# mohsenzakeri/Movi

Measured on AMD Instinct MI355X. Metric: PML query Gbases/s on regular-thresholds index, higher is better.
Workload: dtype u64

## Files before the change

movi_amd/csrc/movi_walk.hpp:

```cpp
#pragma once
#include "movi_device.hpp"

namespace movi {

template <int MODE, typename IdxT, int CLS, int SEP, int SEG, int STG, int AHD, int PSH, int RING>
__global__ __launch_bounds__(256) void pml_kernel_flatp(DevIndex ix, const uint8_t *__restrict__ bases,
                                                       const uint64_t *__restrict__ offs, uint64_t n_reads,
                                                       uint16_t *__restrict__ out, uint8_t *__restrict__ err,
                                                       DevStats *stats, const uint32_t *__restrict__ order,
                                                       ClsArgs cls, SegArgs seg) {
    static_assert(SEG == 0 || CLS == 0, "segments: plain PML");
    static_assert(AHD == 0 || STG == 1, "look-ahead rows: staged reads");
    static_assert(AHD == 0 || AHD == 1 || AHD == 2, "plain rows, look-ahead rows or deep rows");
    static_assert(AHD != 2 || (PSH == 0 && sizeof(IdxT) == 4), "deep rows: tables of fewer than 2^28 rows, no pair-shared gathers");
    static_assert(PSH == 0 || STG == 1, "pair-shared gathers: staged kernels");
    static_assert(RING == 0 || STG == 1, "PMLs out through the LDS ring / as reset masks: staged kernels");
    static_assert(RING != 2 || (CLS == 0 && SEG == 0), "reset masks: plain PML of whole reads");
    enum : uint32_t { sFF = 0, sDown = 1, sUp = 2, sDone = 3 };
    __shared__ uint8_t s_code[256];
    for (int i = threadIdx.x; i < 256; i += blockDim.x) s_code[i] = ix.code_of[i];
    __syncthreads();

    const uint64_t t = (uint64_t)blockIdx.x * blockDim.x + threadIdx.x;
    uint32_t ff_total = 0, scan_total = 0, repo_total = 0, failed = 0, err_total = 0;
    const EndThr ethr = end_thresholds(ix);
    const IdxT r1 = (IdxT)(ix.r - 1), end_row = (IdxT)ix.end_bwt_idx;
    const uint2 row_r1 = load_row<MODE>(ix.rows, r1);
    const uint32_t off0 = row_n<MODE>(row_r1) - 1;

    const bool valid = (SEG == 1 ? (*seg.go != 0u && t < *seg.n_seg) : (t < n_reads && (SEG != 2 || seg.read_fail[t] != 0)));
    const uint64_t rid = (valid && order && SEG == 0) ? order[t] : t;
    const uint64_t beg = valid ? (SEG == 1 ? seg.seg_in[rid] : offs[rid]) : 0;
    const uint32_t len = valid ? (SEG == 1 ? seg.seg_len[rid] : (uint32_t)(offs[rid + 1] - beg)) : 0;
    const uint64_t obeg = (SEG == 1 && valid) ? seg.seg_out[rid] : beg;
    constexpr bool ring = RING == 1;
    constexpr bool msk = RING == 2;
    uint32_t *const M = msk ? reinterpret_cast<uint32_t *>(out) + (((beg + ix.mask_phase) >> 5) + rid) : nullptr;
    uint32_t mk = 0;
    const uint32_t packed_end = len & (ring ? ~15u : ~7u);

    auto load_pair_at = [&](uint64_t e, uint64_t &c0, uint64_t &c1) {
        uint64_t two[2];
        __builtin_memcpy(two, bases + (e >= 16 ? e - 16 : 0), 16);
        c0 = two[1];
        c1 = two[0];
    };
    auto fix_pair = [&](uint64_t e, uint64_t &c0, uint64_t &c1) {
        if (e < 16) {
            const uint32_t sh = 8u * (uint32_t)(16 - e);
            if (sh >= 64) { c0 = c1 << (sh - 64); c1 = 0; }
            else { c0 = (c0 << sh) | (c1 >> (64 - sh)); c1 <<= sh; }
        }
    };
    constexpr uint32_t WN = 4u;
    const IdxT wb_last = (IdxT)(ix.r - WN);
    auto win_base = [&](IdxT nd) -> IdxT {
        const IdxT wb = nd & ~(IdxT)(WN - 1u);
        return wb < wb_last ? wb : wb_last;
    };
    uint2 ahw[4];
    uint4 raw[4];
    uint4 dq[4];
    const uint32_t odd_lane = threadIdx.x & 1u;
    auto fetch = [&](IdxT nd, bool act, uint2 (&w)[4]) {
        if (AHD == 2) {
            const uint32_t q3 = __umulhi((uint32_t)nd, 0xAAAAAAABu) >> 1;
            const uint8_t *at = ix.rows3 + (act ? (uint64_t)q3 * 64u : 0u);
            __builtin_memcpy(&dq[0], at, 16);
            __builtin_memcpy(&dq[1], at + 16, 16);
            __builtin_memcpy(&dq[2], at + 32, 16);
            __builtin_memcpy(&dq[3], at + 48, 16);
            return;
        }
        if (PSH) {
            uint64_t at;
            if (AHD) {
                const IdxT wb = nd & ~(IdxT)3;
                at = wb < wb_last ? (uint64_t)(wb >> 3) * 128u + (uint64_t)((uint32_t)wb & 4u) * 8u : ix.rows2_tail;
            } else {
                at = (uint64_t)win_base(nd) * 8u;
            }
            if (!act) at = 0;
            const uint64_t pat = (uint64_t)pair_swap((uint32_t)at) | ((uint64_t)pair_swap((uint32_t)(at >> 32)) << 32);
            const uint8_t *tab = AHD ? ix.rows2 : ix.rows;
            const uint8_t *pe = tab + (odd_lane ? pat : at) + 16u * odd_lane;
            const uint8_t *po = tab + (odd_lane ? at : pat) + 16u * odd_lane;
            __builtin_memcpy(&raw[0], pe, 16);
            if (AHD) __builtin_memcpy(&raw[2], pe + 64u, 16);
            __builtin_memcpy(&raw[1], po, 16);
            if (AHD) __builtin_memcpy(&raw[3], po + 64u, 16);
            return;
        }
        if (AHD) {
            const IdxT wb = nd & ~(IdxT)3;
            const bool body = wb < wb_last;
            uint64_t at = body ? (uint64_t)(wb >> 3) * 128u + (uint64_t)((uint32_t)wb & 4u) * 8u : ix.rows2_tail;
            if (!act) at = 0;
            load_window<MODE>(ix.rows2 + at, 0, w);
            load_window<MODE>(ix.rows2 + at + 64u, 0, ahw);
        } else {
            load_window<MODE>(ix.rows, (uint64_t)(act ? win_base(nd) : (IdxT)0), w);
        }
    };
    ClsState cs;
    auto finish_read = [&]() {
        if (SEG == 1) {
            SegTot tt;
            tt.ff = ff_total; tt.scan = scan_total; tt.repo = repo_total; tt.flag = failed;
            seg.tot[rid] = tt;
            return;
        }
        if (msk) {
            if (failed) {
                for (uint32_t wd = 0; wd * 32u < len; ++wd) M[wd] = (len - wd * 32u >= 32u) ? 0xFFFFFFFFu : ((1u << (len & 31u)) - 1u);
            } else if (len & 31u) {
                M[len >> 5] = mk;
            }
        } else if (failed && CLS != 2) {
            for (uint32_t i = 0; i < len; ++i) out[obeg + i] = 0;
        }
        if (CLS) cs.store(cls, rid, failed != 0u);
        if (err) err[rid] = (uint8_t)failed;
        err_total += failed ? 1u : 0u;
    };

    uint32_t st = len > 0 ? sFF : sDone;
    IdxT need = r1;
    uint32_t k = 0;
    uint32_t ml = 0, ff_run = 0;
    uint32_t off = off0;
    uint64_t rb = 0, rb2 = 0, nx0 = 0, nx1 = 0;
    if (st != sDone) {
        load_pair_at(beg + len, rb, rb2);
        fix_pair(beg + len, rb, rb2);
    }
    if (!STG && len > 16) load_pair_at(beg + len - 16, nx0, nx1);
    uint32_t a = s_code[(uint32_t)(rb >> 56) & 0xFFu];
    uint4 pk = make_uint4(0, 0, 0, 0), pk_old = pk;
    if (CLS) cs.init(len, cls.bin_width);
    extern __shared__ __align__(16) uint8_t s_stage[];
    uint8_t *const s_ring = s_stage + ix.stage_lds * 64u;
    const uint32_t ring_lane = (threadIdx.x & 63u) * 16u;
    auto ring_put = [&](uint32_t kk, uint32_t val) {
        *reinterpret_cast<uint16_t *>(s_ring + ((kk >> 3) & 3u) * 1024u + ring_lane + (kk & 7u) * 2u) = (uint16_t)val;
    };
    auto ring_flush = [&](uint32_t k0) {
        const uint32_t g = (k0 >> 4) & 1u;
        const uint4 lo = *reinterpret_cast<const uint4 *>(s_ring + (2u * g) * 1024u + ring_lane);
        const uint4 hi = *reinterpret_cast<const uint4 *>(s_ring + (2u * g + 1u) * 1024u + ring_lane);
        uint16_t *dst = out + obeg + (k0 & ~15u);
        __builtin_memcpy(dst, &lo, 16);
        __builtin_memcpy(dst + 8, &hi, 16);
    };
    uint32_t kbase = 0;
    const uint32_t stage_cap = ix.stage_lds;
#ifndef MOVI_STAGE_UNROLL
#define MOVI_STAGE_UNROLL 2
#endif
    constexpr uint32_t kStageUnroll = MOVI_STAGE_UNROLL;
    auto stage_from = [&](uint32_t k0, bool on) {
        uint32_t *S = reinterpret_cast<uint32_t *>(s_stage);
        const uint32_t sl = threadIdx.x & 63u;
        const uint32_t left = (on && len > k0) ? len - k0 : 0u;
        const uint32_t cnt = left < stage_cap ? left : stage_cap;
        for (uint32_t g = 0; wave_any(16u * g < cnt); g += kStageUnroll) {
            uint64_t c0[kStageUnroll], c1[kStageUnroll];
#pragma unroll
            for (uint32_t u = 0; u < kStageUnroll; ++u) {
                const uint64_t e = 16u * (g + u) < cnt ? beg + len - k0 - 16u * (g + u) : 16u;
                load_pair_at(e, c0[u], c1[u]);
            }
#pragma unroll
            for (uint32_t u = 0; u < kStageUnroll; ++u) {
                if (16u * (g + u) < cnt) {
                    const uint64_t e = beg + len - k0 - 16u * (g + u);
                    fix_pair(e, c0[u], c1[u]);
                    const uint64_t r0 = __builtin_bswap64(c0[u]), r1 = __builtin_bswap64(c1[u]);
                    S[(4u * (g + u) + 0u) * 64u + sl] = (uint32_t)r0;
                    S[(4u * (g + u) + 1u) * 64u + sl] = (uint32_t)(r0 >> 32);
                    S[(4u * (g + u) + 2u) * 64u + sl] = (uint32_t)r1;
                    S[(4u * (g + u) + 3u) * 64u + sl] = (uint32_t)(r1 >> 32);
                }
            }
        }
        if (on) kbase = k0;
    };
    auto staged_code = [&](uint32_t slot) -> uint32_t {
        const uint32_t q = slot < stage_cap ? slot : stage_cap - 1u;
        return s_code[s_stage[(q >> 2) * 256u + (threadIdx.x & 63u) * 4u + (q & 3u)]];
    };
    if (STG) stage_from(0u, st != sDone);
    auto top_of_walk = [&](uint32_t cand, uint32_t kidx) -> uint32_t {
        const uint32_t K = ix.kmer_k;
        uint4 e4 = make_uint4(0, 0, 0, 0);
        if (cand) e4 = ix.kmer[kidx];
        const uint32_t use = cand & (e4.y >> 31);
        if (msk) {
            if (use) {
                const uint32_t mask = (e4.y >> 16) & 0xFFFu;
                mk = ~mask & ((1u << K) - 1u);
                k = K;
                ml = (uint32_t)__builtin_clz(~(mask << (32u - K)));
                need = (IdxT)((uint64_t)e4.x | ((uint64_t)(e4.y & 15u) << 32));
                off = (e4.y >> 4) & 0xFFFu;
                ff_total += e4.z;
                scan_total += e4.w;
                repo_total += K - (uint32_t)__popc(mask);
            }
        } else if (use) {
            const uint32_t mask = (e4.y >> 16) & 0xFFFu;
            uint16_t *O = out + obeg;
            uint32_t run = 0;
            for (uint32_t i = 0; i < K; ++i) {
                run = ((mask >> i) & 1u) ? run + 1u : 0u;
                if (CLS) cs.add(run, k, len, cls.bin_width, cls.thr);
                if (CLS == 2) {
                } else if (k >= packed_end) {
                    O[k] = (uint16_t)run;
                } else if (STG && ring) {
                    ring_put(k, run);
                } else {
                    pk.x = (pk.x >> 16) | (pk.y << 16);
                    pk.y = (pk.y >> 16) | (pk.z << 16);
                    pk.z = (pk.z >> 16) | (pk.w << 16);
                    pk.w = (pk.w >> 16) | (run << 16);
                    if ((k & 15) == 7) {
                        if (k + 8 < packed_end) pk_old = pk;
                        else __builtin_memcpy(O + (k - 7), &pk, 16);
                    }
                }
                k += 1;
            }
            ml = run;
            need = (IdxT)((uint64_t)e4.x | ((uint64_t)(e4.y & 15u) << 32));
            off = (e4.y >> 4) & 0xFFFu;
            ff_total += e4.z;
            scan_total += e4.w;
            repo_total += K - (uint32_t)__popc(mask);
        }
        return use;
    };
    if (ix.kmer_k != 0u) {
        const uint32_t K = ix.kmer_k;
        uint32_t kidx = 0, bad = 0;
        for (uint32_t i = 0; i < K; ++i) {
            const uint64_t src = i < 8u ? rb : rb2;
            const uint32_t cc = (uint32_t)s_code[(uint32_t)(src >> (8u * (7u - (i & 7u)))) & 0xFFu] - (uint32_t)SEP;
            bad |= (uint32_t)(cc > 3u);
            kidx |= (cc & 3u) << (2u * i);
        }
        if (top_of_walk((uint32_t)(st != sDone) & (uint32_t)(len > K) & (bad ^ 1u), kidx)) {
            if (K >= 8u) rb = rb2;
            a = s_code[(uint32_t)(rb >> (8u * (7u - (K & 7u)))) & 0xFFu];
        }
    }
    uint32_t a1 = 0xFFu, a2 = 0xFFu;
    if (AHD) a1 = staged_code(k + 1);
    if (AHD == 2) a2 = staged_code(k + 2);
    uint2 w[4];
    fetch(need, st != sDone, w);

    uint32_t lane_steps = 0, wave_steps = 0;
    while (wave_any(st != sDone)) {
        const bool act = st < sDone;
        lane_steps += (uint32_t)act;
        wave_steps += 1;
#if defined(MOVI_PAD_PRE) && MOVI_PAD_PRE > 0
        {
            uint32_t pad = wave_steps;
#pragma unroll
            for (int i = 0; i < MOVI_PAD_PRE; ++i) asm volatile("v_add_u32 %0, %0, %0" : "+v"(pad));
        }
#endif
        struct StepOut {
            uint32_t resolved, match, ffm, lf, mism, scanning, found, down, qf, qn, jump, jdist, landed, landed_down, nf, n, rofff, emit;
            uint32_t dbl, lf2, off1, tpl, lf3, off2, errc, st_next;
            uint64_t j;
            IdxT needf, need_next, j2, j3;
        } R;
        R.tpl = 0; R.lf3 = 0; R.off2 = 0; R.j3 = 0;
        if (AHD == 2) {
            const uint32_t need32 = (uint32_t)need;
            const uint32_t wbase = (__umulhi(need32, 0xAAAAAAABu) >> 1) * 3u;
            const uint32_t r1u = (uint32_t)r1;
            const uint32_t d1a = dq[0].y, d1b = dq[1].z, d1c = dq[2].w;
            const uint32_t n0 = d1a & 0x7FFu, n1w = d1b & 0x7FFu, n2w = d1c & 0x7FFu;
            const uint32_t nm = (uint32_t)(((d1a >> 22) & 7u) != a) | ((uint32_t)(((d1b >> 22) & 7u) != a) << 1) | ((uint32_t)(((d1c >> 22) & 7u) != a) << 2);
            const uint32_t lim = r1u - wbase;
            const uint32_t first_win = (uint32_t)(wbase == 0u);
            uint32_t nd = need32;
            {
                const uint32_t q0 = nd - wbase;
                const uint32_t inw = (uint32_t)(q0 < 3u) & (uint32_t)(st < sDone);
                const uint32_t m0 = q0 == 0u, m1 = q0 <= 1u;
                const uint32_t t1 = m0 ? n0 : 0u, t2 = t1 + (m1 ? n1w : 0u), t3 = t2 + n2w;
                const uint32_t isff = inw & (uint32_t)(st == sFF);
                const uint32_t room = 65534u - (ff_run < 65534u ? ff_run : 65534u);
                uint32_t p0 = isff & m0 & (uint32_t)(off >= t1) & (uint32_t)(0u < lim), p1 = isff & m1 & (uint32_t)(off >= t2) & (uint32_t)(1u < lim),
                         p2 = isff & (uint32_t)(off >= t3) & (uint32_t)(2u < lim);
                uint32_t cf = p0 + p1 + p2;
                if (cf > room) {
                    cf = room;
                    const uint32_t first = m0 ? 0u : (m1 ? 1u : 2u);
                    p0 = p0 & (uint32_t)(first + cf > 0u);
                    p1 = p1 & (uint32_t)(first + cf > 1u);
                    p2 = p2 & (uint32_t)(first + cf > 2u);
                }
                off -= (p2 ? t3 : (p1 ? t2 : (p0 ? t1 : 0u)));
                ff_run += cf;
                const uint32_t dmask = (nm & (lim >= 3u ? 7u : ((1u << lim) - 1u))) >> q0;
                const uint32_t cd = (inw & (uint32_t)(st == sDown)) ? (uint32_t)__builtin_ctz(~dmask | 8u) : 0u;
                const uint32_t umask = ((nm & (first_win ? 6u : 7u)) << (2u - (q0 < 3u ? q0 : 2u))) & 7u;
                const uint32_t cu = (inw & (uint32_t)(st == sUp)) ? (uint32_t)__builtin_clz(((~umask) & 7u) << 29 | 0x10000000u) : 0u;
                scan_total += cd + cu;
                nd = nd + cf + cd - cu;
            }
            need = (IdxT)nd;
            const uint32_t qn = nd - wbase;
            const uint32_t inwin = (uint32_t)(qn < 3u) & (uint32_t)act;
            auto sel3 = [](uint32_t x0, uint32_t x1, uint32_t x2, uint32_t q) { return q == 0u ? x0 : (q == 1u ? x1 : x2); };
            const uint32_t rD0 = sel3(dq[0].x, dq[1].y, dq[2].z, qn), rD1 = sel3(d1a, d1b, d1c, qn);
            const uint32_t n = rD1 & 0x7FFu, c = (rD1 >> 22) & 7u;
            const uint32_t isFF = (uint32_t)(st == sFF) & inwin, isDown = (uint32_t)(st == sDown) & inwin, isUp = (uint32_t)(st == sUp) & inwin;
            const uint32_t ffm = isFF & (uint32_t)(nd < r1u) & (uint32_t)(off >= n);
            const uint32_t ff_over = ffm & (uint32_t)(ff_run + 1 >= 65535u);
            const uint32_t resolved = isFF & (ffm ^ 1u);
            const uint32_t illegal = a == 0xFFu, match = c == a;
            const uint32_t mism = resolved & (illegal ^ 1u) & (match ^ 1u);
            const uint32_t kk = thr_slot(SEP, a, c);
            const uint32_t kc = kk > 2u ? 2u : kk;
            uint32_t thr = ((rD0 >> (28u + kc)) & 1u) ? n : 0u;
            if (SEP) {
                if (mism & (uint32_t)(c == 0u) & (uint32_t)(need != end_row)) thr = separator_threshold(ix, (uint64_t)need, a);
            }
            const uint32_t down = (uint32_t)(off >= ((need == end_row) ? end_threshold(SEP, ethr, a) : thr));
            const uint32_t at_last = nd >= r1u, at_first = nd == 0u;
            const uint32_t repo_edge = mism & (down ? at_last : at_first);
            const uint32_t has = (nm ^ 7u) & (down ? (6u << qn) & 7u : (1u << qn) - 1u);
            const uint32_t found = mism & (uint32_t)(has != 0u) & ix.inwin;
            const uint32_t qf = found ? (down ? (uint32_t)__builtin_ctz(has | 8u) : 31u - (uint32_t)__builtin_clz(has | 1u)) : qn;
            const uint32_t far = mism & (found ^ 1u);
            const uint32_t f0 = sel3(dq[0].x, dq[1].y, dq[2].z, qf), f1 = sel3(d1a, d1b, d1c, qf), f2 = sel3(dq[0].z, dq[1].w, dq[3].x, qf),
                           f3 = sel3(dq[0].w, dq[2].x, dq[3].y, qf), f4 = sel3(dq[1].x, dq[2].y, dq[3].z, qf);
            const uint32_t fx = (dq[3].w >> (10u * (qf < 3u ? qf : 0u))) & 0x3FFu;
            const uint32_t nf = f1 & 0x7FFu, rofff = (f1 >> 11) & 0x7FFu;
            const uint32_t scanning = isDown | isUp;
            const uint32_t hit = scanning & match;
            const uint32_t landed = hit | found;
            const uint32_t landed_down = hit ? isDown : down;
            const uint32_t scan_edge = scanning & (hit ^ 1u) & (isDown ? at_last : at_first);
            const uint32_t emit = (resolved & (illegal | match)) | landed;
            const uint32_t lf = emit & (uint32_t)(k + 1 != len);
            const uint32_t jj = f0 & 0x0FFFFFFFu;
            const uint32_t lf_bad = lf & (uint32_t)(jj >= (uint32_t)ix.r);
            const uint32_t h6 = (f2 >> 28) | ((fx >> 8) << 4);
            const uint32_t hd = __builtin_amdgcn_ubfe(h6, kc + kc, ix.hint_w);
            const uint32_t jump = far & (uint32_t)(hd != 0u);
            const uint32_t jtgt = down ? wbase + 2u + hd : wbase - hd;
            const uint32_t jdist = down ? jtgt - nd : nd - jtgt;
            const uint32_t step_fwd = ffm | (far & down) | (scanning & (hit ^ 1u) & isDown);
            const uint32_t step_back = (far & (down ^ 1u)) | (scanning & (hit ^ 1u) & isUp);
            uint32_t need_next = lf ? jj : (jump ? jtgt : nd + step_fwd - step_back);
            uint32_t st_next = (emit & (lf ^ 1u)) ? sDone : (lf ? sFF : (far ? (down ? sDown : sUp) : st));
            const uint32_t e1n = f3 & 0x7FFu, e1off = (f3 >> 11) & 0x7FFu, e1c = (f1 >> 25) & 7u, jj2 = f2 & 0x0FFFFFFFu;
            const uint32_t e2n = (f3 >> 22) | (((f4 >> 28) & 1u) << 10), e2off = ((f4 >> 29) & 7u) | ((fx & 0xFFu) << 3), e2c = (f1 >> 28) & 7u,
                           jj3 = f4 & 0x0FFFFFFFu;
            const uint32_t off_e = (landed ? (landed_down ? 0u : nf - 1u) : off) + rofff;
            const uint32_t dbl = lf & (uint32_t)(a1 == e1c) & (uint32_t)(off_e < e1n);
            const uint32_t lf2 = dbl & (uint32_t)(k + 2 != len);
            const uint32_t off_e2 = off_e + e1off;
            const uint32_t tpl = lf2 & (uint32_t)(a2 == e2c) & (uint32_t)(off_e2 < e2n);
            const uint32_t lf3 = tpl & (uint32_t)(k + 3 != len);
            need_next = tpl ? (lf3 ? jj3 : nd) : (dbl ? (lf2 ? jj2 : nd) : need_next);
            st_next = tpl ? (lf3 ? sFF : sDone) : (dbl ? (lf2 ? sFF : sDone) : st_next);
            uint32_t errc = kErrNone;
            if (wave_any((ff_over | repo_edge | scan_edge | lf_bad) != 0u)) {
                errc = ff_over ? kErrFastForward
                               : (repo_edge ? (down ? kErrNoRunBelow : kErrNoRunAbove)
                                  : (scan_edge ? (isDown ? kErrNoRunBelow : kErrNoRunAbove)
                                     : (lf_bad ? kErrIdRange : kErrNone)));
                if (errc) { need_next = nd; st_next = sDone; }
            }
            R.resolved = resolved; R.match = match; R.ffm = ffm; R.lf = lf; R.mism = mism; R.scanning = scanning; R.found = found; R.down = down;
            R.qf = qf; R.qn = qn; R.jump = jump; R.jdist = jdist; R.landed = landed; R.landed_down = landed_down; R.nf = nf; R.n = n; R.rofff = rofff;
            R.emit = emit; R.dbl = dbl; R.lf2 = lf2; R.off1 = e1off; R.tpl = tpl; R.lf3 = lf3; R.off2 = e2off; R.errc = errc; R.st_next = st_next;
            R.j = jj; R.needf = (IdxT)(wbase + qf); R.need_next = (IdxT)need_next; R.j2 = (IdxT)jj2; R.j3 = (IdxT)jj3;
        } else {
            if (PSH) {
                pair_assemble(odd_lane, raw[0], raw[1], w);
                if (AHD) pair_assemble(odd_lane, raw[2], raw[3], ahw);
            }
            const IdxT wbase = win_base(need);
            auto hop = [&]() {
                const uint32_t q = (uint32_t)(need - wbase);
                const uint32_t inwin = (uint32_t)(q < WN) & (uint32_t)(st < sDone);
                const uint2 hr = win_sel(w, q);
                const uint32_t hn = row_n<MODE>(hr), hc = row_c<MODE>(hr);
                const uint32_t ffh = inwin & (uint32_t)(st == sFF) & (uint32_t)(need < r1) & (uint32_t)(off >= hn) &
                                     (uint32_t)(ff_run + 1 < 65535u);
                const uint32_t nomatch = hc != a;
                const uint32_t dnh = inwin & (uint32_t)(st == sDown) & nomatch & (uint32_t)(need < r1);
                const uint32_t uph = inwin & (uint32_t)(st == sUp) & nomatch & (uint32_t)(need != 0);
                off = ffh ? off - hn : off;
                ff_run += ffh;
                scan_total += dnh | uph;
                need = need + (IdxT)(ffh + dnh) - (IdxT)uph;
            };
            const uint32_t nm = (uint32_t)(row_c<MODE>(w[0]) != a) | ((uint32_t)(row_c<MODE>(w[1]) != a) << 1) |
                                ((uint32_t)(row_c<MODE>(w[2]) != a) << 2) | ((uint32_t)(row_c<MODE>(w[3]) != a) << 3);
            const uint32_t last_win = (uint32_t)(wbase + 3 == r1);
            const uint32_t first_win = (uint32_t)(wbase == 0);
            auto window_advance = [&]() {
                const uint32_t q0 = (uint32_t)(need - wbase);
                const uint32_t inwin = (uint32_t)(q0 < 4u) & (uint32_t)(st < sDone);
                const uint32_t n0 = row_n<MODE>(w[0]), n1 = row_n<MODE>(w[1]), n2 = row_n<MODE>(w[2]), n3 = row_n<MODE>(w[3]);
                const uint32_t m0 = q0 == 0u, m1 = q0 <= 1u, m2 = q0 <= 2u;
                const uint32_t t1 = m0 ? n0 : 0u, t2 = t1 + (m1 ? n1 : 0u), t3 = t2 + (m2 ? n2 : 0u), t4 = t3 + n3;
                const uint32_t isff = inwin & (uint32_t)(st == sFF);
                const uint32_t p0 = isff & m0 & (uint32_t)(off >= t1), p1 = isff & m1 & (uint32_t)(off >= t2),
                               p2 = isff & m2 & (uint32_t)(off >= t3), p3 = isff & (uint32_t)(off >= t4) & (last_win ^ 1u);
                const uint32_t cf = p0 + p1 + p2 + p3;
                off -= (p3 ? t4 : (p2 ? t3 : (p1 ? t2 : (p0 ? t1 : 0u))));
                ff_run += cf;
                const uint32_t dmask = (nm & (last_win ? 7u : 15u)) >> (q0 & 3u);
                const uint32_t cd = (inwin & (uint32_t)(st == sDown)) ? (uint32_t)__builtin_ctz(~dmask | 16u) : 0u;
                const uint32_t umask = ((nm & (first_win ? 14u : 15u)) << (3u - (q0 & 3u))) & 15u;
                const uint32_t cu = (inwin & (uint32_t)(st == sUp)) ? (uint32_t)__builtin_clz(((~umask) & 15u) << 28 | 0x08000000u) : 0u;
                scan_total += cd + cu;
                need = need + (IdxT)(cf + cd) - (IdxT)cu;
            };
            if (wave_any(st == sFF && ff_run >= 65520u)) {
                for (int h = 0; h < 4; ++h) hop();
            } else {
                window_advance();
            }
            const uint32_t qn = (uint32_t)(need - wbase);
            const uint32_t inwin = (uint32_t)(qn < WN) & (uint32_t)act;
            const uint2 row = win_sel(w, qn);
            const uint32_t n = row_n<MODE>(row), c = row_c<MODE>(row);
            const uint32_t isFF = (uint32_t)(st == sFF) & inwin, isDown = (uint32_t)(st == sDown) & inwin,
                           isUp = (uint32_t)(st == sUp) & inwin;
            const uint32_t ffm = isFF & (uint32_t)(need < r1) & (uint32_t)(off >= n);
            const uint32_t ff_over = ffm & (uint32_t)(ff_run + 1 >= 65535u);
            const uint32_t resolved = isFF & (ffm ^ 1u);
            const uint32_t illegal = a == 0xFFu, match = c == a;
            const uint32_t mism = resolved & (illegal ^ 1u) & (match ^ 1u);
            const uint32_t kk = thr_slot(SEP, a, c);
            uint32_t thr = row_thr<MODE>(row, kk > 2u ? 2u : kk) ? n : 0u;
            if (SEP) {
                if (mism & (uint32_t)(c == 0u) & (uint32_t)(need != end_row)) thr = separator_threshold(ix, (uint64_t)need, a);
            }
            const uint32_t down = (uint32_t)(off >= ((need == end_row) ? end_threshold(SEP, ethr, a) : thr));
            const uint32_t at_last = need >= r1, at_first = need == 0;
            const uint32_t repo_edge = mism & (down ? at_last : at_first);
            const uint32_t has = (nm ^ 15u) & (down ? (14u << (qn & 3u)) & 15u : (1u << (qn & 3u)) - 1u);
            const uint32_t found = mism & (uint32_t)(has != 0u) & ix.inwin;
            const uint32_t qf = found ? (down ? (uint32_t)__builtin_ctz(has | 16u) : 31u - (uint32_t)__builtin_clz(has | 1u)) : qn;
            const uint32_t far = mism & (found ^ 1u);
            const uint2 rowf = win_sel(w, qf);
            const uint32_t nf = row_n<MODE>(rowf), rofff = row_off<MODE>(rowf);
            const IdxT needf = (IdxT)(wbase + qf);
            const uint32_t scanning = isDown | isUp;
            const uint32_t hit = scanning & match;
            const uint32_t landed = hit | found;
            const uint32_t landed_down = hit ? isDown : down;
            const uint32_t scan_edge = scanning & (hit ^ 1u) & (isDown ? at_last : at_first);
            const uint32_t emit = (resolved & (illegal | match)) | landed;
            const uint32_t lf = emit & (uint32_t)(k + 1 != len);
            constexpr bool id32 = AHD != 0 && sizeof(IdxT) == 4;
            uint64_t j = 0;
            if (id32) j = (uint64_t)rowf.x;
            else if (MODE == 6 || lf) j = (AHD && ix.hints) ? (uint64_t)rowf.x : row_id<MODE>(rowf, needf, ix);
            const uint32_t lf_bad = lf & (uint32_t)(j >= ix.r);
            uint2 ah = make_uint2(0u, 0u);
            if (AHD) ah = win_sel(ahw, qf);
            uint32_t jump = 0, jdist = 0;
            IdxT jtgt = 0;
            if (AHD) {
                const uint32_t hbits = (rowf.y >> 28) | ((ah.y >> 21) & 0x3F0u);
                const uint32_t kc = kk > 2u ? 2u : kk;
                const uint32_t hd = __builtin_amdgcn_ubfe(hbits, kc + 2u * kc, ix.hint_w);
                jump = far & (uint32_t)(hd != 0u);
                jtgt = down ? (IdxT)(wbase + 3u + hd) : (IdxT)(wbase - hd);
                jdist = down ? (uint32_t)(jtgt - need) : (uint32_t)(need - jtgt);
            }
            const uint32_t step_fwd = ffm | (far & down) | (scanning & (hit ^ 1u) & isDown);
            const uint32_t step_back = (far & (down ^ 1u)) | (scanning & (hit ^ 1u) & isUp);
            IdxT need_next = lf ? (IdxT)j : (jump ? jtgt : (IdxT)(need + step_fwd - step_back));
            uint32_t st_next = (emit & (lf ^ 1u)) ? sDone : (lf ? sFF : (far ? (down ? sDown : sUp) : st));
            uint32_t dbl = 0, lf2 = 0, off1 = 0;
            IdxT j2 = 0;
            if (AHD) {
                const uint32_t n1 = ah.y & 0x7FFu, c1 = (ah.y >> 22) & 7u;
                const uint32_t off_e = (landed ? (landed_down ? 0u : nf - 1u) : off) + rofff;
                dbl = lf & (ah.y >> 31) & (uint32_t)(a1 == c1) & (uint32_t)(off_e < n1);
                lf2 = dbl & (uint32_t)(k + 2 != len);
                off1 = (ah.y >> 11) & 0x7FFu;
                j2 = (id32 || ix.hints) ? (IdxT)ah.x : (IdxT)((uint64_t)ah.x | ((uint64_t)((ah.y >> 25) & 15u) << 32));
                need_next = dbl ? (lf2 ? j2 : need) : need_next;
                st_next = dbl ? (lf2 ? sFF : sDone) : st_next;
            }
            uint32_t errc = kErrNone;
            if (wave_any((ff_over | repo_edge | scan_edge | lf_bad) != 0u)) {
                errc = ff_over ? kErrFastForward
                               : (repo_edge ? (down ? kErrNoRunBelow : kErrNoRunAbove)
                                  : (scan_edge ? (isDown ? kErrNoRunBelow : kErrNoRunAbove)
                                     : (lf_bad ? kErrIdRange : kErrNone)));
                if (errc) { need_next = need; st_next = sDone; }
            }
            R.resolved = resolved; R.match = match; R.ffm = ffm; R.lf = lf; R.mism = mism; R.scanning = scanning; R.found = found; R.down = down;
            R.qf = qf; R.qn = qn; R.jump = jump; R.jdist = jdist; R.landed = landed; R.landed_down = landed_down; R.nf = nf; R.n = n; R.rofff = rofff;
            R.emit = emit; R.dbl = dbl; R.lf2 = lf2; R.off1 = off1; R.errc = errc; R.st_next = st_next;
            R.j = j; R.needf = needf; R.need_next = need_next; R.j2 = j2;
        }
        const uint32_t resolved = R.resolved, match = R.match, ffm = R.ffm, lf = R.lf, mism = R.mism, scanning = R.scanning, found = R.found,
                       down = R.down, qf = R.qf, qn = R.qn, jump = R.jump, jdist = R.jdist, landed = R.landed, landed_down = R.landed_down,
                       nf = R.nf, n = R.n, rofff = R.rofff, emit = R.emit, dbl = R.dbl, lf2 = R.lf2, off1 = R.off1, tpl = R.tpl, lf3 = R.lf3,
                       off2 = R.off2, errc = R.errc, st_next = R.st_next;
        const uint64_t j = R.j;
        const IdxT needf = R.needf, need_next = R.need_next, j2 = R.j2, j3 = R.j3;
        (void)j3; (void)tpl; (void)lf3; (void)off2;
        fetch(need_next, st_next != sDone, w);
#if defined(MOVI_PAD_POST) && MOVI_PAD_POST > 0
        {
            uint32_t pad = wave_steps;
#pragma unroll
            for (int i = 0; i < MOVI_PAD_POST; ++i) asm volatile("v_add_u32 %0, %0, %0" : "+v"(pad));
        }
#endif
        uint32_t want_nx = 0;
        uint64_t nx_e = 0;
        ml = resolved ? (match ? ml + 1 : 0u) : ml;
        ff_total += resolved ? ff_run : 0u;
        ff_run = lf ? 0u : ff_run + ffm;
        repo_total += mism;
        scan_total += scanning + (found ? (down ? qf - qn : qn - qf) : 0u) + (jump ? jdist - 1u : 0u);
        off = ffm ? off - n : (landed ? (landed_down ? 0u : nf - 1) : off);
        const uint32_t off_pre = off;
        off += lf ? rofff : 0u;
        if (emit) {
            uint16_t *O = out + obeg;
            auto emit_pml = [&](uint32_t mlv) {
                const uint32_t val = mlv > 65535u ? 65535u : mlv;
                if (CLS) cs.add(val, k, len, cls.bin_width, cls.thr);
                if (CLS == 2) {
                } else if (msk) {
                    mk |= (uint32_t)(mlv == 0u) << (k & 31u);
                    if ((k & 31u) == 31u) { M[k >> 5] = mk; mk = 0u; }
                } else if (k >= packed_end) {
                    O[k] = (uint16_t)val;
                } else if (STG && ring) {
                    ring_put(k, val);
                } else {
                    pk.x = (pk.x >> 16) | (pk.y << 16);
                    pk.y = (pk.y >> 16) | (pk.z << 16);
                    pk.z = (pk.z >> 16) | (pk.w << 16);
                    pk.w = (pk.w >> 16) | (val << 16);
                    if ((k & 15) == 7) {
                        if (k + 8 < packed_end) pk_old = pk;
                        else __builtin_memcpy(O + (k - 7), &pk, 16);
                    } else if ((k & 15) == 15) {
                        __builtin_memcpy(O + (k - 15), &pk_old, 16);
                        __builtin_memcpy(O + (k - 7), &pk, 16);
                    }
                }
                k += 1;
            };
            auto seg_record = [&](uint64_t at, uint32_t off_at) {
                if ((k & 31u) == 31u) {
                    SegCkpt ck;
                    ck.idx = at; ck.off = off_at; ck.ml = ml;
                    ck.ff = ff_total; ck.scan = scan_total; ck.repo = repo_total; ck.pad_ = 0;
                    seg.ckpt[(obeg + k) >> 5] = ck;
                }
                if (k + 1 == len) {
                    SegFin fn;
                    fn.idx = at; fn.off = off_at; fn.ml = ml;
                    seg.fin[rid] = fn;
                }
            };
            const uint32_t k_in = k;
            if (SEG == 1) seg_record((uint64_t)needf, off_pre);
            emit_pml(ml);
            if (AHD && dbl) {
                ml += 1;
                if (SEG == 1) seg_record(j, off);
                off += lf2 ? off1 : 0u;
                emit_pml(ml);
            }
            if (AHD == 2 && tpl) {
                ml += 1;
                if (SEG == 1) seg_record((uint64_t)j2, off);
                off += lf3 ? off2 : 0u;
                emit_pml(ml);
            }
            if (STG && CLS != 2 && ring && ((k ^ k_in) & 16u) != 0u) ring_flush(k_in);
            if (STG) {
            } else if (lf) {
                {
                    if ((k & 15) == 8) {
                        rb = rb2;
                    } else if ((k & 15) == 0) {
                        rb = nx0;
                        rb2 = nx1;
                        fix_pair(beg + len - k, rb, rb2);
                        if (k + 16 < len) { want_nx = 1; nx_e = beg + len - k - 16; }
                    }
                    a = s_code[(uint32_t)(rb >> (8 * (7 - (k & 7)))) & 0xFFu];
                }
            }
        }
        if (errc) failed = errc;
        need = need_next;
        st = st_next;
        if (STG) {
            const uint32_t ahead_of = k - kbase;
            const uint32_t out_of = (uint32_t)(st != sDone) &
                                    ((uint32_t)(ahead_of >= stage_cap) | ((uint32_t)(ahead_of + 1u >= stage_cap) & (uint32_t)(k + 1 < len)) |
                                     (AHD == 2 ? ((uint32_t)(ahead_of + 2u >= stage_cap) & (uint32_t)(k + 2 < len)) : 0u));
            if (wave_any(out_of != 0u)) stage_from(k, st != sDone);
            a = staged_code(k - kbase);
            if (AHD) a1 = staged_code(k + 1 - kbase);
            if (AHD == 2) a2 = staged_code(k + 2 - kbase);
        }
        if (want_nx) load_pair_at(nx_e, nx0, nx1);
    }
    if (valid) finish_read();
    if (msk && ix.expand_out != nullptr) {
        __builtin_amdgcn_fence(__ATOMIC_SEQ_CST, "workgroup");
        __syncthreads();
        uint16_t *tile = reinterpret_cast<uint16_t *>(s_stage);
        const uint32_t tile_elems = ix.stage_lds * 32u;
        const uint32_t ln = threadIdx.x & 63u;
        const unsigned long long vb = __ballot(valid);
        if (vb != 0ull) {
            const uint64_t B0 = __shfl(beg, 0, 64);
            const uint64_t B1 = __shfl(beg + len, 63 - __builtin_clzll(vb), 64);
            const uint32_t *Mx = reinterpret_cast<const uint32_t *>(out) + (((beg + ix.mask_phase) >> 5) + rid);
            uint16_t *vec = ix.expand_out;
            uint32_t kx = 0, run = 0, wcur = 0, w0 = 0, w1 = 0;
            const uint64_t endx = beg + len;
            if (valid && len) { w0 = Mx[0]; w1 = Mx[1]; }
            auto one = [&](uint32_t o) {
                if ((kx >> 5) != wcur) { wcur = kx >> 5; w0 = w1; w1 = Mx[wcur + 1]; }
                run = ((w0 >> (kx & 31u)) & 1u) ? 0u : run + 1u;
                tile[o] = (uint16_t)(run > 65535u ? 65535u : run);
                kx += 1;
            };
            for (uint64_t A = B0 & ~7ull; A < B1; A += tile_elems) {
                const uint64_t hi = A + tile_elems < B1 ? A + tile_elems : B1;
                if (valid && kx < len && beg + kx < hi) {
                    uint32_t o = (uint32_t)(beg + kx - A);
                    const uint32_t stop = (uint32_t)((endx < hi ? endx : hi) - A);
                    while (o < stop && (o & 7u)) one(o++);
                    while (o + 8u <= stop) {
                        if ((kx >> 5) != wcur) { wcur = kx >> 5; w0 = w1; w1 = Mx[wcur + 1]; }
                        const uint32_t bits = (uint32_t)((((uint64_t)w1 << 32) | w0) >> (kx & 31u)) & 0xFFu;
                        uint32_t v[8];
#pragma unroll
                        for (uint32_t e = 0; e < 8u; ++e) {
                            run = ((bits >> e) & 1u) ? 0u : run + 1u;
                            v[e] = run > 65535u ? 65535u : run;
                        }
                        *reinterpret_cast<uint4 *>(&tile[o]) = make_uint4(v[0] | (v[1] << 16), v[2] | (v[3] << 16), v[4] | (v[5] << 16), v[6] | (v[7] << 16));
                        o += 8u;
                        kx += 8u;
                    }
                    while (o < stop) one(o++);
                }
                __syncthreads();
                const uint32_t nelem = (uint32_t)(hi - A);
                for (uint32_t g = ln; g * 8u < nelem; g += 64u) {
                    const uint64_t p = A + (uint64_t)g * 8u;
                    const uint4 q = *reinterpret_cast<const uint4 *>(&tile[g * 8u]);
                    if (p >= B0 && p + 8u <= hi) {
                        *reinterpret_cast<uint4 *>(vec + p) = q;
                    } else {
                        const uint32_t x[4] = {q.x, q.y, q.z, q.w};
#pragma unroll
                        for (uint32_t e = 0; e < 8u; ++e)
                            if (p + e >= B0 && p + e < hi) vec[p + e] = (uint16_t)(x[e >> 1] >> (16u * (e & 1u)));
                    }
                }
                __syncthreads();
            }
        }
    }
    if (SEG != 1) {
        const uint32_t ffw = wave_sum(ff_total), scw = wave_sum(scan_total), rpw = wave_sum(repo_total),
                       erw = wave_sum(err_total);
        if ((threadIdx.x & 63) == 0 && stats) {
            if (ffw) atomicAdd(&stats->fast_forwards, (unsigned long long)ffw);
            if (scw) atomicAdd(&stats->scans, (unsigned long long)scw);
            if (rpw) atomicAdd(&stats->repositions, (unsigned long long)rpw);
            if (erw) atomicAdd(&stats->errors, (unsigned long long)erw);
        }
    }
    const uint32_t lsw = wave_sum(lane_steps);
    if ((threadIdx.x & 63) == 0 && stats) {
        atomicAdd(&stats->lane_steps, (unsigned long long)lsw);
        atomicAdd(&stats->wave_steps, (unsigned long long)wave_steps);
    }
}

template <typename IdxT, int SEG, int CLS, int SEP, int STG, int AHD, int PSH, int RING>
static hipError_t walk_go(const WalkLaunch &L, LaunchInfo *info) {
    auto kern = pml_kernel_flatp<6, IdxT, CLS, SEP, SEG, STG, AHD, PSH, RING>;
    if (L.dyn_lds > 65536) {
        const hipError_t ea = hipFuncSetAttribute(reinterpret_cast<const void *>(kern), hipFuncAttributeMaxDynamicSharedMemorySize, (int)L.dyn_lds);
        if (ea != hipSuccess) return ea;
    }
    hipLaunchKernelGGL(kern, L.grid, L.block, L.dyn_lds, L.stream, L.ix, L.bases, L.offs, L.n, L.out, L.err, L.stats, L.order, L.cls, L.seg);
    char name[96];
    snprintf(name, sizeof(name), "pml_kernel_flatp<6, %s, %d, %d, %d, %d, %d, %d, %d>", sizeof(IdxT) == 4 ? "unsigned int" : "unsigned long",
             CLS, SEP, SEG, STG, AHD, PSH, RING);
    if (info) snprintf(info->kernel, sizeof(info->kernel), "%s", name);
    note_walk_launch(name);
    return hipGetLastError();
}
template <typename IdxT, int SEG, int CLS, int SEP>
static hipError_t walk_pick(const WalkLaunch &L, LaunchInfo *info) {
    if (!L.stg) return walk_go<IdxT, SEG, CLS, SEP, 0, 0, 0, 0>(L, info);
    if (L.ahd == 2) {
        if constexpr (sizeof(IdxT) == 4) {
            if (L.ring == 2) {
                if constexpr (SEG == 0 && CLS == 0) return walk_go<IdxT, 0, 0, SEP, 1, 2, 0, 2>(L, info);
                else return hipErrorInvalidValue;
            }
            return L.ring ? walk_go<IdxT, SEG, CLS, SEP, 1, 2, 0, 1>(L, info) : walk_go<IdxT, SEG, CLS, SEP, 1, 2, 0, 0>(L, info);
        } else {
            return hipErrorInvalidValue;
        }
    }
    if (L.ring == 2) {
        if constexpr (SEG == 0 && CLS == 0) {
            switch ((L.ahd ? 2 : 0) | (L.psh ? 1 : 0)) {
            case 0: return walk_go<IdxT, 0, 0, SEP, 1, 0, 0, 2>(L, info);
            case 1: return walk_go<IdxT, 0, 0, SEP, 1, 0, 1, 2>(L, info);
            case 2: return walk_go<IdxT, 0, 0, SEP, 1, 1, 0, 2>(L, info);
            default: return walk_go<IdxT, 0, 0, SEP, 1, 1, 1, 2>(L, info);
            }
        } else {
            return hipErrorInvalidValue;
        }
    }
    switch ((L.ahd ? 4 : 0) | (L.psh ? 2 : 0) | (L.ring ? 1 : 0)) {
    case 0: return walk_go<IdxT, SEG, CLS, SEP, 1, 0, 0, 0>(L, info);
    case 1: return walk_go<IdxT, SEG, CLS, SEP, 1, 0, 0, 1>(L, info);
    case 2: return walk_go<IdxT, SEG, CLS, SEP, 1, 0, 1, 0>(L, info);
    case 3: return walk_go<IdxT, SEG, CLS, SEP, 1, 0, 1, 1>(L, info);
    case 4: return walk_go<IdxT, SEG, CLS, SEP, 1, 1, 0, 0>(L, info);
    case 5: return walk_go<IdxT, SEG, CLS, SEP, 1, 1, 0, 1>(L, info);
    case 6: return walk_go<IdxT, SEG, CLS, SEP, 1, 1, 1, 0>(L, info);
    default: return walk_go<IdxT, SEG, CLS, SEP, 1, 1, 1, 1>(L, info);
    }
}
template <typename IdxT, int SEG>
static hipError_t walk_dispatch(const WalkLaunch &L, LaunchInfo *info) {
    if (SEG != 0 || L.cls_mode == 0) return L.sep ? walk_pick<IdxT, SEG, 0, 1>(L, info) : walk_pick<IdxT, SEG, 0, 0>(L, info);
    if (SEG == 0 && L.cls_mode == 1) return L.sep ? walk_pick<IdxT, 0, 1, 1>(L, info) : walk_pick<IdxT, 0, 1, 0>(L, info);
    if (SEG == 0) return L.sep ? walk_pick<IdxT, 0, 2, 1>(L, info) : walk_pick<IdxT, 0, 2, 0>(L, info);
    return hipErrorInvalidValue;
}

}
```

Measured before the change: 87.20.

## Streamline staged code lookups, mask emission and FF clamp in PML walk

Several micro-optimizations of the per-step walk loop. Staged base codes for a, a1 and a2 are now read with one or two LDS word loads plus alignbyte instead of separate byte loads with clamping, and the stage capacity is reduced by 8 so the look-ahead never runs past the staged slots. Restaging checks are skipped entirely when no lane's read exceeds the stage capacity. The mask output path is handled as a separate branch that advances k by emit+dbl+tpl at once, the deep-row window base reuses the quotient computed in fetch, and the FF-run saturation clamp is guarded by a wave-wide check so it runs only near overflow.

```diff
diff --git a/movi_amd/csrc/movi_walk.hpp b/movi_amd/csrc/movi_walk.hpp
--- a/movi_amd/csrc/movi_walk.hpp
+++ b/movi_amd/csrc/movi_walk.hpp
@@ -62,9 +62,11 @@
     uint4 raw[4];
     uint4 dq[4];
     const uint32_t odd_lane = threadIdx.x & 1u;
+    uint32_t win3 = 0;
     auto fetch = [&](IdxT nd, bool act, uint2 (&w)[4]) {
         if (AHD == 2) {
             const uint32_t q3 = __umulhi((uint32_t)nd, 0xAAAAAAABu) >> 1;
+            win3 = q3;
             const uint8_t *at = ix.rows3 + (act ? (uint64_t)q3 * 64u : 0u);
             __builtin_memcpy(&dq[0], at, 16);
             __builtin_memcpy(&dq[1], at + 16, 16);
@@ -135,7 +137,6 @@
         fix_pair(beg + len, rb, rb2);
     }
     if (!STG && len > 16) load_pair_at(beg + len - 16, nx0, nx1);
-    uint32_t a = s_code[(uint32_t)(rb >> 56) & 0xFFu];
     uint4 pk = make_uint4(0, 0, 0, 0), pk_old = pk;
     if (CLS) cs.init(len, cls.bin_width);
     extern __shared__ __align__(16) uint8_t s_stage[];
@@ -153,7 +154,7 @@
         __builtin_memcpy(dst + 8, &hi, 16);
     };
     uint32_t kbase = 0;
-    const uint32_t stage_cap = ix.stage_lds;
+    const uint32_t stage_cap = STG ? ix.stage_lds - 8u : 0u;
 #ifndef MOVI_STAGE_UNROLL
 #define MOVI_STAGE_UNROLL 2
 #endif
@@ -185,11 +186,17 @@
         }
         if (on) kbase = k0;
     };
-    auto staged_code = [&](uint32_t slot) -> uint32_t {
-        const uint32_t q = slot < stage_cap ? slot : stage_cap - 1u;
-        return s_code[s_stage[(q >> 2) * 256u + (threadIdx.x & 63u) * 4u + (q & 3u)]];
+    uint32_t a = STG ? 0xFFu : (uint32_t)s_code[(uint32_t)(rb >> 56) & 0xFFu], a1 = 0xFFu, a2 = 0xFFu;
+    auto staged_codes = [&](uint32_t slot) {
+        const uint32_t *S = reinterpret_cast<const uint32_t *>(s_stage) + (slot >> 2) * 64u + (threadIdx.x & 63u);
+        const uint32_t lo = S[0];
+        const uint32_t v = AHD ? __builtin_amdgcn_alignbyte(S[64], lo, slot & 3u) : lo >> (8u * (slot & 3u));
+        a = s_code[v & 0xFFu];
+        if (AHD) a1 = s_code[(v >> 8) & 0xFFu];
+        if (AHD == 2) a2 = s_code[(v >> 16) & 0xFFu];
     };
     if (STG) stage_from(0u, st != sDone);
+    const bool rolls = STG && wave_any(len > stage_cap);
     auto top_of_walk = [&](uint32_t cand, uint32_t kidx) -> uint32_t {
         const uint32_t K = ix.kmer_k;
         uint4 e4 = make_uint4(0, 0, 0, 0);
@@ -251,12 +258,10 @@
         }
         if (top_of_walk((uint32_t)(st != sDone) & (uint32_t)(len > K) & (bad ^ 1u), kidx)) {
             if (K >= 8u) rb = rb2;
-            a = s_code[(uint32_t)(rb >> (8u * (7u - (K & 7u)))) & 0xFFu];
-        }
-    }
-    uint32_t a1 = 0xFFu, a2 = 0xFFu;
-    if (AHD) a1 = staged_code(k + 1);
-    if (AHD == 2) a2 = staged_code(k + 2);
+            if (!STG) a = s_code[(uint32_t)(rb >> (8u * (7u - (K & 7u)))) & 0xFFu];
+        }
+    }
+    if (STG) staged_codes(k);
     uint2 w[4];
     fetch(need, st != sDone, w);
 
@@ -281,7 +286,7 @@
         R.tpl = 0; R.lf3 = 0; R.off2 = 0; R.j3 = 0;
         if (AHD == 2) {
             const uint32_t need32 = (uint32_t)need;
-            const uint32_t wbase = (__umulhi(need32, 0xAAAAAAABu) >> 1) * 3u;
+            const uint32_t wbase = win3 * 3u;
             const uint32_t r1u = (uint32_t)r1;
             const uint32_t d1a = dq[0].y, d1b = dq[1].z, d1c = dq[2].w;
             const uint32_t n0 = d1a & 0x7FFu, n1w = d1b & 0x7FFu, n2w = d1c & 0x7FFu;
@@ -295,16 +300,18 @@
                 const uint32_t m0 = q0 == 0u, m1 = q0 <= 1u;
                 const uint32_t t1 = m0 ? n0 : 0u, t2 = t1 + (m1 ? n1w : 0u), t3 = t2 + n2w;
                 const uint32_t isff = inw & (uint32_t)(st == sFF);
-                const uint32_t room = 65534u - (ff_run < 65534u ? ff_run : 65534u);
                 uint32_t p0 = isff & m0 & (uint32_t)(off >= t1) & (uint32_t)(0u < lim), p1 = isff & m1 & (uint32_t)(off >= t2) & (uint32_t)(1u < lim),
                          p2 = isff & (uint32_t)(off >= t3) & (uint32_t)(2u < lim);
                 uint32_t cf = p0 + p1 + p2;
-                if (cf > room) {
-                    cf = room;
-                    const uint32_t first = m0 ? 0u : (m1 ? 1u : 2u);
-                    p0 = p0 & (uint32_t)(first + cf > 0u);
-                    p1 = p1 & (uint32_t)(first + cf > 1u);
-                    p2 = p2 & (uint32_t)(first + cf > 2u);
+                if (wave_any(st == sFF && ff_run >= 65520u)) {
+                    const uint32_t room = 65534u - (ff_run < 65534u ? ff_run : 65534u);
+                    if (cf > room) {
+                        cf = room;
+                        const uint32_t first = m0 ? 0u : (m1 ? 1u : 2u);
+                        p0 = p0 & (uint32_t)(first + cf > 0u);
+                        p1 = p1 & (uint32_t)(first + cf > 1u);
+                        p2 = p2 & (uint32_t)(first + cf > 2u);
+                    }
                 }
                 off -= (p2 ? t3 : (p1 ? t2 : (p0 ? t1 : 0u)));
                 ff_run += cf;
@@ -538,15 +545,20 @@
         off = ffm ? off - n : (landed ? (landed_down ? 0u : nf - 1) : off);
         const uint32_t off_pre = off;
         off += lf ? rofff : 0u;
-        if (emit) {
+        if (msk) {
+            const uint32_t cnt = emit + dbl + tpl;
+            const uint32_t k_in = k;
+            mk |= (emit & (uint32_t)(ml == 0u)) << (k_in & 31u);
+            ml += dbl + tpl;
+            off += (lf2 ? off1 : 0u) + (lf3 ? off2 : 0u);
+            k = k_in + cnt;
+            if ((k_in ^ k) & 32u) { M[k_in >> 5] = mk; mk = 0u; }
+        } else if (emit) {
             uint16_t *O = out + obeg;
             auto emit_pml = [&](uint32_t mlv) {
                 const uint32_t val = mlv > 65535u ? 65535u : mlv;
                 if (CLS) cs.add(val, k, len, cls.bin_width, cls.thr);
                 if (CLS == 2) {
-                } else if (msk) {
-                    mk |= (uint32_t)(mlv == 0u) << (k & 31u);
-                    if ((k & 31u) == 31u) { M[k >> 5] = mk; mk = 0u; }
                 } else if (k >= packed_end) {
                     O[k] = (uint16_t)val;
                 } else if (STG && ring) {
@@ -614,14 +626,14 @@
         need = need_next;
         st = st_next;
         if (STG) {
-            const uint32_t ahead_of = k - kbase;
-            const uint32_t out_of = (uint32_t)(st != sDone) &
-                                    ((uint32_t)(ahead_of >= stage_cap) | ((uint32_t)(ahead_of + 1u >= stage_cap) & (uint32_t)(k + 1 < len)) |
-                                     (AHD == 2 ? ((uint32_t)(ahead_of + 2u >= stage_cap) & (uint32_t)(k + 2 < len)) : 0u));
-            if (wave_any(out_of != 0u)) stage_from(k, st != sDone);
-            a = staged_code(k - kbase);
-            if (AHD) a1 = staged_code(k + 1 - kbase);
-            if (AHD == 2) a2 = staged_code(k + 2 - kbase);
+            if (rolls) {
+                const uint32_t ahead_of = k - kbase;
+                const uint32_t out_of = (uint32_t)(st != sDone) &
+                                        ((uint32_t)(ahead_of >= stage_cap) | ((uint32_t)(ahead_of + 1u >= stage_cap) & (uint32_t)(k + 1 < len)) |
+                                         (AHD == 2 ? ((uint32_t)(ahead_of + 2u >= stage_cap) & (uint32_t)(k + 2 < len)) : 0u));
+                if (wave_any(out_of != 0u)) stage_from(k, st != sDone);
+            }
+            staged_codes(k - kbase);
         }
         if (want_nx) load_pair_at(nx_e, nx0, nx1);
     }
```

After: 87.73, median of 6. No clear change (+0.6%).
